# sttts/kcp

Measured on AMD Instinct MI355X. Metric: object-pair diffs/sec (whole node) + achieved HBM GB/s, 10M objs/100k clusters, higher is better.
Workload: dtype u8; 1 GPU; config3: 10000000 pairs / 100000 logical clusters node-wide, 5% mutated (40% ConfigMap/Secret, 40% Deployment, 20% CRD); pairs_per_rank=10000000, passes_in_flight=2, parallelism=shard-by-logical-cluster x1 (LPT)

## Files before the change

include/gpudiff.h:

```cpp
#ifndef GPUDIFF_H
#define GPUDIFF_H

#include <stddef.h>
#include <stdint.h>

#include "gpudiff_format.h"

#ifdef __cplusplus
extern "C" {
#endif

#define GPUDIFF_ABI_VERSION 6

enum {
    GPUDIFF_OK = 0,
    GPUDIFF_E_INVAL = -1,
    GPUDIFF_E_NOMEM = -2,
    GPUDIFF_E_DEVICE = -3,
    GPUDIFF_E_NODEVICE = -4,
    GPUDIFF_E_CAPACITY = -5,
    GPUDIFF_E_STATE = -6,
    GPUDIFF_E_DECODE = -7,
    GPUDIFF_E_NOTFOUND = -8,
};
// ... 166 lines not shown
int gpudiff_dbatch_create(gpudiff_ctx* ctx, uint64_t pool_bytes, uint64_t max_pairs,
                          gpudiff_dbatch** out);
int gpudiff_dbatch_create_view(gpudiff_ctx* ctx, const gpudiff_dbatch* base, gpudiff_dbatch** out);
int gpudiff_dbatch_append(gpudiff_ctx* ctx, gpudiff_dbatch* db, const gpudiff_hbatch* hb);
int gpudiff_dbatch_reset(gpudiff_ctx* ctx, gpudiff_dbatch* db);
int gpudiff_dbatch_stats_get(const gpudiff_dbatch* db, gpudiff_batch_stats* st);
int gpudiff_dbatch_device_view(const gpudiff_dbatch* db, gpudiff_device_view* v);
#define GPUDIFF_EXPORT_COUNTS 0u
#define GPUDIFF_EXPORT_SPEC_IDS 1u
#define GPUDIFF_EXPORT_STATUS_IDS 2u
#define GPUDIFF_EXPORT_DIRTY_IDS 3u
#define GPUDIFF_EXPORT_FLAGS 4u
int gpudiff_dbatch_export(gpudiff_ctx* ctx, const gpudiff_dbatch* db, uint32_t what, void* dst_device,
                          uint64_t max_elems, uint64_t known_count);
int gpudiff_dbatch_bind_gather(gpudiff_ctx* ctx, gpudiff_dbatch* db, void* send_dev, uint32_t cap_spec,
                               uint32_t cap_status);
int gpudiff_dbatch_result_slot(gpudiff_ctx* ctx, gpudiff_dbatch* db, uint32_t slot);
int gpudiff_dbatch_read_pool(gpudiff_ctx* ctx, const gpudiff_dbatch* db, uint64_t off, void* dst,
                             uint64_t bytes);
void gpudiff_dbatch_free(gpudiff_ctx* ctx, gpudiff_dbatch* db);

int gpudiff_cluster_bytes(const gpudiff_pair_row* rows, size_t n, uint32_t n_clusters, uint64_t* out);
int gpudiff_shard_lpt(const uint64_t* weights, uint32_t n_clusters, uint32_t world, int32_t* owner);

int gpudiff_diff(gpudiff_ctx* ctx, gpudiff_dbatch* db, gpudiff_ticket* ticket);
int gpudiff_wait(gpudiff_ctx* ctx, gpudiff_ticket ticket, gpudiff_result* res);
void gpudiff_result_release(gpudiff_ctx* ctx, gpudiff_result* res);
int gpudiff_last_timings(gpudiff_ctx* ctx, gpudiff_timings* t);
int gpudiff_timing_reset(gpudiff_ctx* ctx);
int gpudiff_sync(gpudiff_ctx* ctx);
typedef struct gpudiff_pass_stats {
    uint64_t passes;
    uint64_t small_passes;
    uint64_t small_redone;
    uint64_t redo_arena, redo_deep, redo_paths;
    uint64_t readback_rounds;
} gpudiff_pass_stats;
int gpudiff_pass_stats_get(gpudiff_ctx* ctx, gpudiff_pass_stats* out);

int gpudiff_submit(gpudiff_ctx* ctx, const gpudiff_json_pair* pairs, size_t n,
                   gpudiff_ticket* ticket);

typedef struct gpudiff_store gpudiff_store;

typedef struct gpudiff_event {
    uint32_t slot;
// ... 220 lines not shown
```

include/gpudiff_format.h:

```cpp
#ifndef GPUDIFF_FORMAT_H
#define GPUDIFF_FORMAT_H

#include <stdint.h>

#ifdef __HIPCC__
#define GPUDIFF_HD __host__ __device__
#else
#define GPUDIFF_HD
#endif

#define GPUDIFF_TAG_NULL 0u
#define GPUDIFF_TAG_FALSE 1u
#define GPUDIFF_TAG_TRUE 2u
#define GPUDIFF_TAG_INT 3u
#define GPUDIFF_TAG_FLOAT 4u
#define GPUDIFF_TAG_STR 5u
#define GPUDIFF_TAG_EOBJ 6u
#define GPUDIFF_TAG_EARR 7u

#define GPUDIFF_INLINE_MAX 8u
#define GPUDIFF_PATH_HASH_BITS 32u

#define GPUDIFF_OBJ_HAS_STATUS 0x1u
#define GPUDIFF_OBJ_DECODE_ERR 0x2u
#define GPUDIFF_OBJ_FRESH 0x4u
#define GPUDIFF_TAB_INDEX 0x8000000000000000ull
#define GPUDIFF_TAB_NONE 0xFFFFFFFFu
GPUDIFF_HD static inline uint64_t gpudiff_tab_bytes(uint32_t n, uint64_t key_bytes) {
    return (24ull * n + key_bytes + 127u) & ~(uint64_t)127u;
}

#define GPUDIFF_OBJ_SEED_SHIFT 8u

#ifdef __cplusplus
extern "C" {
#endif

typedef struct gpudiff_pair_row {
    uint64_t off_a;
    uint64_t off_b;
    uint32_t spec_l_a, spec_l_b;
    uint32_t spec_ar_a, spec_ar_b;
    uint32_t stat_l_a, stat_l_b;
    uint32_t stat_ar_a, stat_ar_b;
    uint32_t flags_a, flags_b;
    uint32_t pair_id, cluster_id;
} gpudiff_pair_row;

GPUDIFF_HD static inline uint64_t gpudiff_seg_bytes(uint32_t l, uint32_t arena) {
    return (uint64_t)l * 16u + (uint64_t)arena;
}

#define GPUDIFF_BLOB_ALIGN 128u
GPUDIFF_HD static inline uint64_t gpudiff_blob_body(uint32_t sl, uint32_t sar, uint32_t tl, uint32_t tar) {
    return (gpudiff_seg_bytes(sl, sar) + gpudiff_seg_bytes(tl, tar) + (GPUDIFF_BLOB_ALIGN - 1u)) &
           ~(uint64_t)(GPUDIFF_BLOB_ALIGN - 1u);
}

GPUDIFF_HD static inline uint64_t gpudiff_pair_compare_bytes(const gpudiff_pair_row* r) {
    const uint64_t al = GPUDIFF_BLOB_ALIGN - 1u;
    uint64_t per = 0;
    if ((r->flags_a | r->flags_b) & GPUDIFF_OBJ_DECODE_ERR) return sizeof(gpudiff_pair_row) + 1u;
    {
        const int spec_sz = r->spec_l_a == r->spec_l_b && r->spec_ar_a == r->spec_ar_b;
        const int stat_sz = (r->flags_b & GPUDIFF_OBJ_HAS_STATUS) && r->stat_l_a == r->stat_l_b &&
                            r->stat_ar_a == r->stat_ar_b;
        const uint64_t seg_s = gpudiff_seg_bytes(r->spec_l_a, r->spec_ar_a);
        const uint64_t seg_t = gpudiff_seg_bytes(r->stat_l_a, r->stat_ar_a);
        if (spec_sz && stat_sz) per = (seg_s + seg_t + al) & ~al;
        else if (spec_sz) per = (r->stat_l_a | r->stat_l_b | r->stat_ar_a | r->stat_ar_b) ? seg_s : (seg_s + al) & ~al;
        else if (stat_sz) per = seg_t;
    }
    return sizeof(gpudiff_pair_row) + 1u + 2u * per;
}

#define GPUDIFF_PD_ERR 0x01u
#define GPUDIFF_PD_SPEC_EQ 0x02u
#define GPUDIFF_PD_STAT_EQ 0x04u
#define GPUDIFF_PD_HAS_ST_B 0x08u
#define GPUDIFF_PD_HAS_ST_A 0x10u
#define GPUDIFF_PD_SEED 0x20u
#define GPUDIFF_PD_NO_STAT 0x40u
#define GPUDIFF_PD_SIZE_BITS 19u
#define GPUDIFF_PD_SIZE_MAX 0x7FFFFu
#define GPUDIFF_PD_ESCAPE 0xFFFFFFFFu

typedef struct gpudiff_pair_desc {
    uint32_t w[4];
} gpudiff_pair_desc;

typedef struct gpudiff_pair_geom {
    uint64_t off_a, off_b;
    uint32_t n1, n2, adj_a, adj_b;
    uint32_t bits;
} gpudiff_pair_geom;

GPUDIFF_HD static inline gpudiff_pair_geom gpudiff_pair_geom_of(uint64_t off_a, uint64_t off_b, uint32_t seg_a,
                                                                uint32_t seg_b, uint32_t seg_t, uint32_t bits) {
    gpudiff_pair_geom g;
    const int ok = !(bits & GPUDIFF_PD_ERR);
    const int spec_sz = (bits & GPUDIFF_PD_SPEC_EQ) != 0u;
    const int stat_sz = (bits & GPUDIFF_PD_HAS_ST_B) && (bits & GPUDIFF_PD_STAT_EQ);
    const uint32_t r128 = (seg_a + seg_t + 127u) & ~127u;
    g.off_a = off_a;
    g.off_b = off_b;
    g.n1 = (ok && spec_sz) ? ((!stat_sz && (bits & GPUDIFF_PD_NO_STAT)) ? ((seg_a + 127u) & ~127u) : seg_a) >> 4 : 0u;
    g.n2 = (ok && stat_sz) ? (spec_sz ? r128 - seg_a : seg_t) >> 4 : 0u;
    g.adj_a = seg_a - 16u * g.n1;
    g.adj_b = seg_b - 16u * g.n1;
    g.bits = bits;
    return g;
}

GPUDIFF_HD static inline uint32_t gpudiff_pair_row_bits(const gpudiff_pair_row* r) {
    return (((r->flags_a | r->flags_b) & GPUDIFF_OBJ_DECODE_ERR) ? GPUDIFF_PD_ERR : 0u) |
           ((r->spec_l_a == r->spec_l_b && r->spec_ar_a == r->spec_ar_b) ? GPUDIFF_PD_SPEC_EQ : 0u) |
           ((r->stat_l_a == r->stat_l_b && r->stat_ar_a == r->stat_ar_b) ? GPUDIFF_PD_STAT_EQ : 0u) |
           ((r->flags_b & GPUDIFF_OBJ_HAS_STATUS) ? GPUDIFF_PD_HAS_ST_B : 0u) |
           ((r->flags_a & GPUDIFF_OBJ_HAS_STATUS) ? GPUDIFF_PD_HAS_ST_A : 0u) |
           (((r->flags_a >> GPUDIFF_OBJ_SEED_SHIFT) & 0xFFu) ? GPUDIFF_PD_SEED : 0u) |
           ((r->stat_l_a | r->stat_l_b | r->stat_ar_a | r->stat_ar_b) == 0u ? GPUDIFF_PD_NO_STAT : 0u);
}

GPUDIFF_HD static inline gpudiff_pair_geom gpudiff_pair_row_geom(const gpudiff_pair_row* r) {
    return gpudiff_pair_geom_of(r->off_a, r->off_b, (uint32_t)gpudiff_seg_bytes(r->spec_l_a, r->spec_ar_a),
                                (uint32_t)gpudiff_seg_bytes(r->spec_l_b, r->spec_ar_b),
                                (uint32_t)gpudiff_seg_bytes(r->stat_l_a, r->stat_ar_a), gpudiff_pair_row_bits(r));
}

GPUDIFF_HD static inline gpudiff_pair_desc gpudiff_pair_desc_pack(const gpudiff_pair_row* r) {
    gpudiff_pair_desc d;
    const uint64_t sa = gpudiff_seg_bytes(r->spec_l_a, r->spec_ar_a), sb = gpudiff_seg_bytes(r->spec_l_b, r->spec_ar_b);
    const uint64_t st = gpudiff_seg_bytes(r->stat_l_a, r->stat_ar_a);
    const uint32_t bits = gpudiff_pair_row_bits(r);
    const uint64_t size_max = (uint64_t)GPUDIFF_PD_SIZE_MAX << 4;
    const int fits = ((r->off_a | r->off_b) & (GPUDIFF_BLOB_ALIGN - 1u)) == 0u && (r->off_a >> 7) <= 0xFFFFFFFFull &&
                     (r->off_b >> 7) <= 0xFFFFFFFFull && ((sa | sb | st) & 15u) == 0u && sa <= size_max &&
                     sb <= size_max && st <= size_max &&
                     ((uint32_t)(r->stat_l_a + r->stat_l_b) == 0u) == ((bits & GPUDIFF_PD_NO_STAT) != 0u);
    if (!fits) {
        d.w[0] = d.w[1] = d.w[2] = d.w[3] = GPUDIFF_PD_ESCAPE;
        return d;
    }
    {
        const uint64_t zw = (sa >> 4) | ((sb >> 4) << GPUDIFF_PD_SIZE_BITS) | ((st >> 4) << (2u * GPUDIFF_PD_SIZE_BITS)) |
                            ((uint64_t)bits << (3u * GPUDIFF_PD_SIZE_BITS));
        d.w[0] = (uint32_t)(r->off_a >> 7);
        d.w[1] = (uint32_t)(r->off_b >> 7);
        d.w[2] = (uint32_t)zw;
        d.w[3] = (uint32_t)(zw >> 32);
    }
    return d;
}

GPUDIFF_HD static inline int gpudiff_pair_desc_is_escape(uint32_t w3) { return w3 == GPUDIFF_PD_ESCAPE; }

GPUDIFF_HD static inline gpudiff_pair_geom gpudiff_pair_desc_unpack(uint32_t w0, uint32_t w1, uint32_t w2, uint32_t w3) {
    const uint64_t zw = ((uint64_t)w3 << 32) | w2;
    return gpudiff_pair_geom_of((uint64_t)w0 << 7, (uint64_t)w1 << 7, (w2 & GPUDIFF_PD_SIZE_MAX) << 4,
                                ((uint32_t)(zw >> GPUDIFF_PD_SIZE_BITS) & GPUDIFF_PD_SIZE_MAX) << 4,
                                ((w3 >> (2u * GPUDIFF_PD_SIZE_BITS - 32u)) & GPUDIFF_PD_SIZE_MAX) << 4,
                                w3 >> (3u * GPUDIFF_PD_SIZE_BITS - 32u));
}

GPUDIFF_HD static inline uint32_t gpudiff_meta(uint32_t tag, uint32_t len) { return (len << 3) | tag; }
GPUDIFF_HD static inline uint32_t gpudiff_meta_tag(uint32_t m) { return m & 7u; }
GPUDIFF_HD static inline uint32_t gpudiff_meta_len(uint32_t m) { return m >> 3; }
GPUDIFF_HD static inline int gpudiff_meta_is_long(uint32_t m) {
    return gpudiff_meta_tag(m) == GPUDIFF_TAG_STR && gpudiff_meta_len(m) > GPUDIFF_INLINE_MAX;
}
GPUDIFF_HD static inline uint32_t gpudiff_meta_arena(uint32_t m) {
    return gpudiff_meta_is_long(m) ? ((gpudiff_meta_len(m) - GPUDIFF_INLINE_MAX + 3u) & ~3u) : 0u;
}
GPUDIFF_HD static inline uint32_t gpudiff_arena_bytes(uint32_t sum) { return (sum + 15u) & ~15u; }

#ifdef __cplusplus
}
#endif
#endif
```

kcp_amd/csrc/api.cpp:

```cpp
#include <hip/hip_runtime.h>
#include <stdlib.h>
#include <string.h>

#include <algorithm>
#include <array>
#include <atomic>
#include <memory>
#include <mutex>
#include <new>
#include <string>
#include <thread>
#include <unordered_map>
#include <vector>

#include "../../include/gpudiff.h"
#include "encoder.h"
#include "dstore.h"
#include "engine.h"
#include "kernels.h"
#include "small_pass.h"
#include "xxh64.h"

using namespace gd;

// ... 543 lines not shown
    d->res_slot = slot;
    return GPUDIFF_OK;
}

int gpudiff_dbatch_read_pool(gpudiff_ctx* c, const gpudiff_dbatch* d, uint64_t off, void* dst, uint64_t bytes) {
    if (!c || !d || (!dst && bytes)) return GPUDIFF_E_INVAL;
    if (d->base) d = d->base;
    int rc = set_device(c);
    if (rc) return rc;
    if (off > d->pool_used || bytes > d->pool_used - off) return GPUDIFF_E_INVAL;
    HIPCHK(hipStreamSynchronize(c->stream));
    if (bytes) HIPCHK(hipMemcpy(dst, d->pool + off, bytes, hipMemcpyDeviceToHost));
    return GPUDIFF_OK;
}

int gpudiff_cluster_bytes(const gpudiff_pair_row* rows, size_t n, uint32_t n_clusters, uint64_t* out) {
    if ((n && !rows) || (n_clusters && !out)) return GPUDIFF_E_INVAL;
    for (size_t i = 0; i < n; i++)
        if (rows[i].cluster_id >= n_clusters) return GPUDIFF_E_INVAL;
    for (size_t i = 0; i < n; i++) out[rows[i].cluster_id] += gpudiff_pair_compare_bytes(&rows[i]);
    return GPUDIFF_OK;
}

int gpudiff_shard_lpt(const uint64_t* weights, uint32_t n_clusters, uint32_t world, int32_t* owner) {
    if (world == 0 || world > 0x7FFFFFFFu || (n_clusters && (!weights || !owner))) return GPUDIFF_E_INVAL;
    try {
        std::vector<uint32_t> order(n_clusters);
        for (uint32_t c = 0; c < n_clusters; c++) order[c] = c;
        std::sort(order.begin(), order.end(), [&](uint32_t x, uint32_t y) {
            return weights[x] != weights[y] ? weights[x] > weights[y] : x < y;
        });
        std::vector<std::pair<uint64_t, uint32_t>> heap;
        heap.reserve(world);
        for (uint32_t r = 0; r < world; r++) heap.emplace_back(0, r);
        auto gt = [](const std::pair<uint64_t, uint32_t>& a, const std::pair<uint64_t, uint32_t>& b) { return a > b; };
        std::make_heap(heap.begin(), heap.end(), gt);
        for (uint32_t c : order) {
            std::pop_heap(heap.begin(), heap.end(), gt);
            auto& top = heap.back();
            owner[c] = (int32_t)top.second;
            top.first += weights[c];
            std::push_heap(heap.begin(), heap.end(), gt);
        }
    } catch (const std::bad_alloc&) {
        return GPUDIFF_E_NOMEM;
    }
// ... 498 lines not shown
```

kcp_amd/csrc/encoder.cpp:

```cpp
#include "encoder.h"

#include <string.h>

#include <algorithm>

#include "xxh64.h"

namespace gd {

static const Node* find_member(const Node& obj, const char* key, uint32_t klen) {
    if (obj.t != J_OBJ) return nullptr;
    for (uint32_t i = 0; i < obj.n; i++) {
        const Member& m = obj.u.mem[i];
        if (m.klen == klen && memcmp(m.k, key, klen) == 0) return &m.v;
    }
    return nullptr;
}

static inline void push_key(std::string& p, const char* k, uint32_t n) {
    char hdr[5];
    hdr[0] = 0x01;
    memcpy(hdr + 1, &n, 4);
    p.append(hdr, 5);
    p.append(k, n);
// ... 237 lines not shown
    seg(o.spec, sl, sar);
    seg(o.stat, tl, tar);
    pool_align(pool);
}

void PairEncoder::encode_flat(FlatObject* fa, FlatObject* fb, uint32_t pair_id, uint32_t cluster_id,
                              std::vector<uint8_t>& pool, gpudiff_pair_row& row) {
    memset(&row, 0, sizeof(row));
    row.pair_id = pair_id;
    row.cluster_id = cluster_id;
    uint32_t seed = 0;
    if (!fa || !fb || !assign_seed(*fa, *fb, &seed)) {
        decode_errors++;
        pool_align(pool);
        row.off_a = row.off_b = pool.size();
        row.flags_a = row.flags_b = GPUDIFF_OBJ_DECODE_ERR;
        return;
    }
    if (seed) reseeded++;
    write_blob(*fa, pool, &row.off_a, &row.spec_l_a, &row.spec_ar_a, &row.stat_l_a, &row.stat_ar_a);
    write_blob(*fb, pool, &row.off_b, &row.spec_l_b, &row.spec_ar_b, &row.stat_l_b, &row.stat_ar_b);
    row.flags_a = fa->flags | (seed << GPUDIFF_OBJ_SEED_SHIFT);
    row.flags_b = fb->flags | (seed << GPUDIFF_OBJ_SEED_SHIFT);
}

void PairEncoder::encode_nodes(const Node* a, const Node* b, uint32_t pair_id, uint32_t cluster_id,
                               std::vector<uint8_t>& pool, gpudiff_pair_row& row) {
    FlatObject* fa = nullptr;
    FlatObject* fb = nullptr;
    if (a && b) {
        flatten_object(*a, flat_a);
        flatten_object(*b, flat_b);
        fa = &flat_a;
        fb = &flat_b;
    }
    encode_flat(fa, fb, pair_id, cluster_id, pool, row);
}

void PairEncoder::encode_json(const uint8_t* a, size_t alen, const uint8_t* b, size_t blen, uint32_t pair_id,
                              uint32_t cluster_id, std::vector<uint8_t>& pool, gpudiff_pair_row& row) {
    arena_a.reset();
    arena_b.reset();
    Node na, nb;
    bool oka = a && parser.parse_object(a, alen, arena_a, &na) && !decodes_as_list(na);
    bool okb = oka && b && parser.parse_object(b, blen, arena_b, &nb) && !decodes_as_list(nb);
    encode_nodes(oka ? &na : nullptr, okb ? &nb : nullptr, pair_id, cluster_id, pool, row);
// ... 229 lines not shown
```

kcp_amd/csrc/kernels.hip:

```cpp
#include <hip/hip_runtime.h>
#include <stdint.h>

#include "../../include/gpudiff.h"
#include "join_dev.h"
#include "kernels.h"
#include "stream_paths.h"
#include "wave_dev.h"
#include "xxh64.h"

namespace gd {


constexpr uint32_t SCAN_TILE = 4096;

struct V4 {
    uint32_t x, y, z, w;
};
__device__ __forceinline__ uint32_t vadd(uint32_t a, uint32_t b) { return a + b; }
__device__ __forceinline__ V4 vadd(const V4& a, const V4& b) {
    return V4{a.x + b.x, a.y + b.y, a.z + b.z, sat_add(a.w, b.w)};
}
template <class V> __device__ __forceinline__ V vzero() { return V{}; }
__device__ __forceinline__ uint32_t vshfl(uint32_t v, uint32_t src) { return shfl32(v, src); }
__device__ __forceinline__ V4 vshfl(const V4& v, uint32_t src) {
// ... 65 lines not shown
    V run = vadd(vadd(wpre[0], wpre[1]), vadd(wpre[2], wpre[3]));
    if (base_in) run = vadd(run, *base_in);
    for (uint32_t w = 0; w < (t >> 6); w++) run = vadd(run, wsum[w]);
    const V excl_thread = vshfl(incl, lane_id() ? lane_id() - 1 : 0);
    if (lane_id()) run = vadd(run, excl_thread);
#pragma unroll
    for (int k = 0; k < 16; k++) {
        const uint32_t i = base + t * 16 + k;
        if (i < n) out[i] = run;
        run = vadd(run, v[k]);
    }
    if (blockIdx.x == last && t == 255) {
        *total = run;
        if (write_terminal) out[n] = run;
        if (mirror) mirror_store(mirror, run);
    }
}


struct StreamLog {
    uint32_t cnt[2][64];
    uint32_t ent[2][64][kSpLogCap];
    uint32_t first[64], n1[64];
};

__device__ uint32_t stream_region(const RegionView& A, const RegionView& B, uint64_t seg, const uint32_t* ent,
                                  uint32_t c, uint32_t g0, uint8_t region_bit, uint64_t* __restrict__ out_h,
                                  uint8_t* __restrict__ out_k, uint32_t out_base, uint32_t lane, bool* weq_all) {
    const uint32_t nc = 4u * c;
    const uint32_t e = lane < nc ? ent[lane >> 2] - sp_entry(g0, 0u) : 0u;
    const bool cand = lane < nc && ((sp_entry_dwords(e) >> (lane & 3u)) & 1u);
    const uint64_t b = sp_entry_byte(e, lane & 3u);
    const SpWhere w = sp_classify(b, A.L);
    if (ballot(cand && (b >= seg || w.cls == SP_KEY))) return kSpRefuse;
    uint32_t leaf = w.idx;
    const bool ar = cand && w.cls == SP_ARENA;
    if (ballot(ar)) {
        bool found = false;
        uint32_t run = 0;
        for (uint32_t i0 = 0; i0 < A.L; i0 += 64u) {
            const uint32_t n = min(64u, A.L - i0);
            const uint32_t as = lane < n ? meta_arena(A.metas[i0 + lane]) : 0u;
            const uint32_t inc = wave_incl_scan(as);
            const uint32_t tot = shfl32(inc, 63);
            const uint32_t rel = w.idx - run;
            uint32_t o = 0;
#pragma unroll
            for (uint32_t s = 32; s >= 1; s >>= 1)
                if (shfl32(inc, o + s - 1u) <= rel) o += s;
            if (ar && !found && w.idx >= run && rel < tot) {
                leaf = i0 + o;
                found = true;
            }
// ... 25 lines not shown
        xb = B.vals[leaf];
    }
    if (ballot(uq && meta_arena(ma) != meta_arena(mb))) return kSpRefuse;
    if (uq) {
        out_h[out_base + rank] = key;
        out_k[out_base + rank] = region_bit | GPUDIFF_PATH_CHANGED;
    }
    *weq_all = !ballot(uq && !wire_equal_number(ma, xa, mb, xb));
    return popc64(um);
}

__device__ uint32_t stream_pair(const gpudiff_pair_row& r, uint32_t f, const uint8_t* pool, uint64_t mask,
                                uint64_t* out_h, uint8_t* out_k, uint32_t base, uint32_t lane, uint32_t* noop,
                                const StreamLog* log, uint32_t k, bool log_ok, uint32_t* n_stream) {
    uint32_t n = 0;
    bool spec_weq = true, stat_weq = true;
    if (f & F_JSPEC) {
        RegionView A = region_view(pool, r.off_a, r.spec_l_a, r.spec_ar_a, false, r.spec_l_a);
        RegionView B = region_view(pool, r.off_b, r.spec_l_b, r.spec_ar_b, false, r.spec_l_b);
        const uint32_t c = log_ok ? uni(log->cnt[0][k]) : 0u;
        const uint32_t g0 = uni(log->first[k]);
        uint32_t got = kSpRefuse;
        if (c >= 1u && c <= kSpLogCap)
            got = stream_region(A, B, seg_bytes(r.spec_l_a, r.spec_ar_a), log->ent[0][k], c, g0, 0, out_h, out_k, base + n,
                                lane, &spec_weq);
        if (got == kSpRefuse) got = join_region<true>(A, B, 0, out_h, out_k, base + n, lane, &spec_weq);
        else (*n_stream)++;
        n += got;
    }
    if (f & F_JSTAT) {
        RegionView A = region_view(pool, r.off_a, r.spec_l_a, r.spec_ar_a, true, r.stat_l_a);
        RegionView B = region_view(pool, r.off_b, r.spec_l_b, r.spec_ar_b, true, r.stat_l_b);
        const uint32_t c = log_ok ? uni(log->cnt[1][k]) : 0u;
        const uint32_t g0 = uni(log->first[k]) + uni(log->n1[k]);
        uint32_t got = kSpRefuse;
        if (c >= 1u && c <= kSpLogCap)
            got = stream_region(A, B, seg_bytes(r.stat_l_a, r.stat_ar_a), log->ent[1][k], c, g0,
                                GPUDIFF_PATH_REGION_STATUS, out_h, out_k, base + n, lane, &stat_weq);
        if (got == kSpRefuse)
            got = join_region<true>(A, B, GPUDIFF_PATH_REGION_STATUS, out_h, out_k, base + n, lane, &stat_weq);
        else (*n_stream)++;
        n += got;
    }
    const bool stat_ok = stat_weq && (!(f & F_SENT) || !(r.flags_a & GPUDIFF_OBJ_HAS_STATUS));
    *noop = (((f & F_SPEC) && spec_weq) ? NOOP_SPEC : 0u) | (((f & F_STATUS) && stat_ok) ? NOOP_STATUS : 0u);
    if (f & F_SENT) {
        if (lane == 0) {
            out_h[base + n] = status_sentinel_hash((r.flags_a >> GPUDIFF_OBJ_SEED_SHIFT) & 0xFFu, mask);
            out_k[base + n] = GPUDIFF_PATH_REGION_STATUS | GPUDIFF_PATH_STATUS_ABSENT;
        }
        n += 1;
    }
    return n;
}

__device__ __forceinline__ bool place_deferred(uint32_t d, uint64_t so, uint32_t cap, uint64_t scratch_cap,
                                               uint32_t* __restrict__ slot_owner) {
    if (so > scratch_cap || cap > scratch_cap - so) return false;
    const uint32_t b0 = (uint32_t)((so + kJoinSlice - 1u) / kJoinSlice);
    const uint32_t b1 = (uint32_t)((so + cap + kJoinSlice - 1u) / kJoinSlice);
// ... 361 lines not shown
    const uint32_t nwaves = (gridDim.x * blockDim.x) >> 6;
    const uint32_t sub_shift = sub_arg & 0xFFu, tail_q = (sub_arg >> 8) & 0xFFu;
    const uint32_t tail_ish = min(sub_shift + 1u, 3u);
    const uint32_t wbase = arena_off + wave * arena_stride;
    uint32_t used = 0;
    bool deferred = false;
    const uint64_t sent0 = status_sentinel_hash(0, mask);
    __shared__ HelpSlot help_slots[HELP ? 4 : 1];
    [[maybe_unused]] HelpSlot* const my = &help_slots[HELP ? (threadIdx.x >> 6) : 0];
    if constexpr (HELP) {
        if (lane == 0) {
            my->gen = my->cursor = my->total = my->helpers = my->p0 = my->cnt = 0u;
            my->mis_s = my->mis_t = 0ull;
        }
        __syncthreads();
    }
    [[maybe_unused]] StreamLog* slog = nullptr;
    [[maybe_unused]] uint32_t n_stream = 0;
    if constexpr (!HELP) {
        __shared__ StreamLog stream_logs[4];
        slog = &stream_logs[uni(threadIdx.x >> 6)];
    }
    auto stream_pass = [&](uint32_t base, uint32_t total, uint32_t incl, uint32_t first, uint32_t n1, uint32_t adj_a,
                           uint32_t adj_b, uint64_t off_a, uint64_t off_b, uint64_t& mis_s, uint64_t& mis_t) {
        u32x4 va[U], vb[U];
        uint32_t own[U];
        bool st[U], act[U];
#pragma unroll
        for (int u = 0; u < U; u++) {
            const uint32_t g = base + (uint32_t)u * 64u + lane;
            act[u] = g < total;
            uint32_t o = 0;
#pragma unroll
            for (uint32_t s = 32; s >= 1; s >>= 1)
                if (shfl32(incl, o + s - 1u) <= g) o += s;
            const uint32_t k = g - shfl32(first, o);
            st[u] = k >= shfl32(n1, o);
            const uint32_t xa = shfl32(adj_a, o), xb = shfl32(adj_b, o);
            const uint64_t oa = shfl64(off_a, o), ob = shfl64(off_b, o);
            own[u] = HELP ? o : o | (st[u] ? 64u : 0u);
            const uint64_t rel = 16ull * k;
            if (act[u]) {
                va[u] = __builtin_nontemporal_load((const u32x4*)(pool + oa + rel + (st[u] ? xa : 0u)));
                vb[u] = __builtin_nontemporal_load((const u32x4*)(pool + ob + rel + (st[u] ? xb : 0u)));
            }
        }
        if constexpr (HELP) {
#pragma unroll
            for (int u = 0; u < U; u++) {
                uint64_t m = ballot(act[u] && neq16(va[u], vb[u]));
                while (m) {
                    const uint32_t j = (uint32_t)__builtin_ctzll(m);
                    m &= m - 1;
                    const uint64_t bit = 1ull << (uint32_t)__builtin_amdgcn_readlane((int)own[u], (int)j);
                    if (__builtin_amdgcn_readlane((int)(st[u] ? 1 : 0), (int)j)) mis_t |= bit;
                    else mis_s |= bit;
                }
            }
        } else {
            uint32_t info[U];
#pragma unroll
            for (int u = 0; u < U; u++) {
                const uint32_t dw = (va[u].x != vb[u].x ? 1u : 0u) | (va[u].y != vb[u].y ? 2u : 0u) |
                                    (va[u].z != vb[u].z ? 4u : 0u) | (va[u].w != vb[u].w ? 8u : 0u);
                info[u] = own[u] | (act[u] ? dw << 7 : 0u);
            }
#pragma unroll
// ... 68 lines not shown
            if (!HELP && it < n_main && lane == 0) tk = atomicAdd(ctr, 1u);
            continue;
        }
        const uint32_t cnt = min(per, n - p0);
        const bool valid = lane < cnt;
        u32x4 v0 = {0, 0, 0, 0}, v1 = v0, v2 = v0, v3 = v0;
        [[maybe_unused]] u32x4 dv = v0;
        if constexpr (DESC) {
            if (valid) dv = *(const u32x4*)(desc + p0 + lane);
        } else if (valid) {
            const u32x4* rp = (const u32x4*)(rows + p0 + lane);
            v0 = rp[0];
            v1 = rp[1];
            v2 = rp[2];
            v3 = rp[3];
        }
        if constexpr (PROF) {
            tp_r = wall_clock64();
            tp_rows += tp_r - tp_i;
        }
        uint64_t off_a, off_b;
        bool err, spec_sz, has_st_b, stat_sz;
        uint32_t n1, n2, adj_a, adj_b;
        [[maybe_unused]] uint32_t dbits = 0;
        constexpr uint32_t kPdRow = 0x80u;
        if constexpr (DESC) {
            gpudiff_pair_geom g = gpudiff_pair_desc_unpack(dv.x, dv.y, dv.z, dv.w);
            if (valid && gpudiff_pair_desc_is_escape(dv.w)) {
                const gpudiff_pair_row r = rows[p0 + lane];
                g = gpudiff_pair_row_geom(&r);
                g.bits |= kPdRow;
            }
            dbits = g.bits;
            off_a = g.off_a, off_b = g.off_b;
            err = valid && (dbits & GPUDIFF_PD_ERR) != 0u;
            spec_sz = (dbits & GPUDIFF_PD_SPEC_EQ) != 0u;
            has_st_b = (dbits & GPUDIFF_PD_HAS_ST_B) != 0u;
            stat_sz = has_st_b && (dbits & GPUDIFF_PD_STAT_EQ) != 0u;
            n1 = valid ? g.n1 : 0u, n2 = valid ? g.n2 : 0u;
            adj_a = g.adj_a, adj_b = g.adj_b;
        } else {
            off_a = ((uint64_t)v0.y << 32) | v0.x, off_b = ((uint64_t)v0.w << 32) | v0.z;
            err = valid && ((v3.x | v3.y) & GPUDIFF_OBJ_DECODE_ERR) != 0u;
            const bool ok = valid && !err;
            spec_sz = v1.x == v1.y && v1.z == v1.w;
            has_st_b = (v3.y & GPUDIFF_OBJ_HAS_STATUS) != 0u;
            stat_sz = has_st_b && v2.x == v2.y && v2.z == v2.w;
            const uint32_t seg_a = (uint32_t)seg_bytes(v1.x, v1.z), seg_b = (uint32_t)seg_bytes(v1.y, v1.w);
            const uint32_t seg_t = (uint32_t)seg_bytes(v2.x, v2.z);
            const uint32_t r128 = ((seg_a + seg_t + 127u) & ~127u);
            const bool no_stat = (v2.x | v2.y | v2.z | v2.w) == 0u;
            n1 = (ok && spec_sz) ? ((!stat_sz && no_stat) ? ((seg_a + 127u) & ~127u) : seg_a) >> 4 : 0u;
            n2 = (ok && stat_sz) ? (spec_sz ? r128 - seg_a : seg_t) >> 4 : 0u;
            adj_a = seg_a - 16u * n1, adj_b = seg_b - 16u * n1;
        }
        const uint32_t tot = n1 + n2;
        const uint32_t incl = wave_incl_scan(tot);
        const uint32_t total = uni(shfl32(incl, 63));
        const uint32_t first = incl - tot;
        uint64_t mis_s = 0, mis_t = 0;
        [[maybe_unused]] uint64_t tp_s0 = 0;
        if constexpr (PROF) {
            tp_s0 = wall_clock64();
// ... 10 lines not shown
                __hip_atomic_store(&my->mis_t, 0ull, __ATOMIC_RELAXED, __HIP_MEMORY_SCOPE_WORKGROUP);
                lds_st(&my->cursor, 64u * U);
                lds_st(&my->gen, lds_ld(&my->gen) + 1u);
            }
            for (uint32_t base = 0; base < total;) {
                uint32_t nb = 0;
                if (lane == 0) nb = lds_add(&my->cursor, 64u * U);
                stream_pass(base, total, incl, first, n1, adj_a, adj_b, off_a, off_b, mis_s, mis_t);
                base = uni(__builtin_amdgcn_readlane(nb, 0));
            }
            if (lane == 0) {
                lds_or64(&my->mis_s, mis_s);
                lds_or64(&my->mis_t, mis_t);
            }
            while (uni(lds_ld(&my->helpers)) != 0u) __builtin_amdgcn_s_sleep(1);
            const uint64_t ms = lds_ld64(&my->mis_s), mt = lds_ld64(&my->mis_t);
            mis_s = ((uint64_t)uni((uint32_t)(ms >> 32)) << 32) | uni((uint32_t)ms);
            mis_t = ((uint64_t)uni((uint32_t)(mt >> 32)) << 32) | uni((uint32_t)mt);
        } else {
            slog->cnt[0][lane] = 0u;
            slog->cnt[1][lane] = 0u;
            slog->first[lane] = first;
            slog->n1[lane] = n1;
            uint32_t pass = 0;
            for (uint32_t base = 0; base < total; base += 64u * U, pass++) {
                stream_pass(base, total, incl, first, n1, adj_a, adj_b, off_a, off_b, mis_s, mis_t);
                if (pass == 0 && it < n_main && lane == 0) tk = atomicAdd(ctr, 1u);
            }
            if (pass == 0 && it < n_main && lane == 0) tk = atomicAdd(ctr, 1u);
        }
        [[maybe_unused]] uint64_t tp_s1 = 0;
        if constexpr (PROF) {
            tp_s1 = wall_clock64();
            tp_stream += tp_s1 - tp_s0;
        }
        if constexpr (DESC) {
            v3.x = ((dbits & GPUDIFF_PD_HAS_ST_A) ? GPUDIFF_OBJ_HAS_STATUS : 0u) |
                   ((dbits & GPUDIFF_PD_SEED) ? 1u << GPUDIFF_OBJ_SEED_SHIFT : 0u);
            const bool sd = !spec_sz || ((mis_s >> lane) & 1ull), td = !stat_sz || ((mis_t >> lane) & 1ull);
            const bool plain_sent = !sd && !has_st_b && (dbits & GPUDIFF_PD_NO_STAT) && !(dbits & (GPUDIFF_PD_SEED | kPdRow));
            if (valid && !err && (sd || td) && !plain_sent) {
                const uint32_t* rp = (const uint32_t*)(rows + p0 + lane);
                const uint2 ls = *(const uint2*)(rp + 4), lt = *(const uint2*)(rp + 8);
                v1.x = ls.x, v1.y = ls.y;
                v2.x = lt.x, v2.y = lt.y;
                v3.x = rp[12];
            }
        }
        uint32_t myflag = 0, mycap = 0, mysrc = 0, mycnt = 0, mynoop = 0;
// ... 516 lines not shown
```

kcp_amd/csrc/stream_paths.h:

```cpp
#pragma once
#include <stdint.h>

#include "../../include/gpudiff_format.h"

#if defined(__HIPCC__)
#define GD_SP_HD __host__ __device__
#else
#define GD_SP_HD
#endif

namespace gd {

constexpr uint32_t kSpLogCap = 4;
constexpr uint32_t kSpMaxLeaves = 64;
constexpr uint32_t kSpRefuse = 0xFFFFFFFFu;

GD_SP_HD inline uint32_t sp_entry(uint32_t chunk, uint32_t dwords) { return (chunk << 4) | (dwords & 15u); }
GD_SP_HD inline uint32_t sp_entry_dwords(uint32_t e) { return e & 15u; }
GD_SP_HD inline uint64_t sp_entry_byte(uint32_t e, uint32_t d) { return 16ull * (e >> 4) + 4u * d; }

GD_SP_HD inline uint32_t sp_meta_arena(uint32_t m) {
    return ((m & 7u) == GPUDIFF_TAG_STR && (m >> 3) > GPUDIFF_INLINE_MAX) ? (((m >> 3) - GPUDIFF_INLINE_MAX + 3u) & ~3u)
                                                                          : 0u;
}

enum SpClass : uint32_t { SP_VAL = 0, SP_KEY = 1, SP_META = 2, SP_ARENA = 3 };
struct SpWhere {
    uint32_t cls;
    uint32_t idx;
};
GD_SP_HD inline SpWhere sp_classify(uint64_t b, uint32_t L) {
    const uint64_t l = L;
    if (b < 8u * l) return SpWhere{SP_VAL, (uint32_t)(b >> 3)};
    if (b < 12u * l) return SpWhere{SP_KEY, (uint32_t)((b - 8u * l) >> 2)};
    if (b < 16u * l) return SpWhere{SP_META, (uint32_t)((b - 12u * l) >> 2)};
    return SpWhere{SP_ARENA, (uint32_t)(b - 16u * l)};
}

GD_SP_HD inline uint32_t sp_arena_owner(const uint32_t* metas, uint32_t L, uint32_t ao) {
    uint32_t off = 0;
    for (uint32_t i = 0; i < L; i++) {
        const uint32_t n = sp_meta_arena(metas[i]);
// ... 35 lines not shown
```

kcp_amd/gpudiff.py:

```python
from __future__ import annotations

import ctypes as C
import json
import os
from dataclasses import dataclass
from typing import Any, Iterable, List, Optional, Sequence, Tuple, Union

import numpy as np

from . import buildinfo

_HERE = os.path.dirname(os.path.abspath(__file__))
LIB_PATH = os.path.join(_HERE, "libgpudiff.so")

ABI_VERSION = 6
OK = 0
E_INVAL, E_NOMEM, E_DEVICE, E_NODEVICE, E_CAPACITY, E_STATE, E_DECODE, E_NOTFOUND = range(-1, -9, -1)

SPEC_DIRTY, STATUS_DIRTY, DECODE_ERROR, SPEC_NOOP, STATUS_NOOP = 0x1, 0x2, 0x4, 0x8, 0x10
PATH_CHANGED, PATH_ADDED, PATH_REMOVED, PATH_STATUS_ABSENT = 0, 1, 2, 3
PATH_REGION_STATUS = 0x80
TAG_NULL, TAG_FALSE, TAG_TRUE, TAG_INT, TAG_FLOAT, TAG_STR, TAG_EOBJ, TAG_EARR = range(8)
VALUE_ABSENT = 0xFF
OPT_TIMING = 0x1
OPT_DEVICE_ENCODE = 0x2000000
OPT_PATH_STRINGS = 0x8000000
OPT_PATH_VALUES = 0x80000000
OPT_K2_ROWS = 0x40
OPT_ARENA_SHIFT = 21
OPT_SMALL_PASS = 0x20000000
SMALL_PASS_MAX_PAIRS = 4096
SMALL_PASS_MAX_PATHS = 32768
DEVICE_CURRENT, DEVICE_NONE = -1, -2

PATH_HASH_BITS = 32
OBJ_HAS_STATUS, OBJ_DECODE_ERR, OBJ_FRESH, OBJ_SEED_SHIFT = 0x1, 0x2, 0x4, 8
STORE_DEVICE_ENCODE = 0x1
EXPORT_COUNTS, EXPORT_SPEC_IDS, EXPORT_STATUS_IDS, EXPORT_DIRTY_IDS, EXPORT_FLAGS = range(5)


class GpuDiffError(RuntimeError):
    def __init__(self, code: int, where: str):
        self.code = code
        super().__init__("%s: %s (%d)" % (where, _lib.gpudiff_strerror(code).decode(), code))


class Opts(C.Structure):
    _fields_ = [("device", C.c_int32), ("encode_threads", C.c_uint32), ("stream", C.c_void_p),
                ("flags", C.c_uint32), ("path_hash_bits", C.c_uint32)]


class JsonPair(C.Structure):
    _fields_ = [("old_json", C.c_void_p), ("old_len", C.c_size_t), ("new_json", C.c_void_p),
                ("new_len", C.c_size_t), ("pair_id", C.c_uint32), ("cluster_id", C.c_uint32)]


JSON_PAIR_DTYPE = np.dtype([("old_json", "<u8"), ("old_len", "<u8"), ("new_json", "<u8"), ("new_len", "<u8"),
                            ("pair_id", "<u4"), ("cluster_id", "<u4")])
assert JSON_PAIR_DTYPE.itemsize == C.sizeof(JsonPair)
# ... 241 lines not shown
SIGNATURES = [
    ("gpudiff_strerror", C.c_char_p, [C.c_int]),
    ("gpudiff_abi_version", C.c_int, []),
    ("gpudiff_build_id", C.c_char_p, []),
    ("gpudiff_device_count", C.c_int, [C.POINTER(C.c_int)]),
    ("gpudiff_open", C.c_int, [C.POINTER(Opts), C.POINTER(_P)]),
    ("gpudiff_close", None, [_P]),
    ("gpudiff_encode_pairs", C.c_int, [_P, C.POINTER(JsonPair), C.c_size_t, C.POINTER(_P)]),
    ("gpudiff_hbatch_info_get", C.c_int, [_P, C.POINTER(HBatchInfo)]),
    ("gpudiff_hbatch_free", None, [_P, _P]),
    ("gpudiff_dbatch_create", C.c_int, [_P, C.c_uint64, C.c_uint64, C.POINTER(_P)]),
    ("gpudiff_dbatch_append", C.c_int, [_P, _P, _P]),
    ("gpudiff_dbatch_reset", C.c_int, [_P, _P]),
    ("gpudiff_dbatch_stats_get", C.c_int, [_P, C.POINTER(BatchStats)]),
    ("gpudiff_dbatch_device_view", C.c_int, [_P, C.POINTER(DeviceView)]),
    ("gpudiff_dbatch_read_pool", C.c_int, [_P, _P, C.c_uint64, C.c_void_p, C.c_uint64]),
    ("gpudiff_dbatch_export", C.c_int, [_P, _P, C.c_uint32, C.c_void_p, C.c_uint64, C.c_uint64]),
    ("gpudiff_dbatch_free", None, [_P, _P]),
    ("gpudiff_dbatch_bind_gather", C.c_int, [_P, _P, C.c_void_p, C.c_uint32, C.c_uint32]),
    ("gpudiff_dbatch_result_slot", C.c_int, [_P, _P, C.c_uint32]),
    ("gpudiff_dbatch_create_view", C.c_int, [_P, _P, C.POINTER(_P)]),
    ("gpudiff_cluster_bytes", C.c_int, [C.c_void_p, C.c_size_t, C.c_uint32, C.c_void_p]),
    ("gpudiff_shard_lpt", C.c_int, [C.c_void_p, C.c_uint32, C.c_uint32, C.c_void_p]),
    ("gpudiff_diff", C.c_int, [_P, _P, C.POINTER(C.c_uint64)]),
    ("gpudiff_wait", C.c_int, [_P, C.c_uint64, C.POINTER(Result)]),
    ("gpudiff_result_release", None, [_P, C.POINTER(Result)]),
    ("gpudiff_result_path_strings", C.c_int, [_P, C.POINTER(Result), C.POINTER(PathStringsC)]),
    ("gpudiff_path_strings_stats_get", C.c_int, [_P, C.POINTER(PathStats)]),
    ("gpudiff_result_path_values", C.c_int, [_P, C.POINTER(Result), C.POINTER(PathValuesC)]),
    ("gpudiff_path_values_stats_get", C.c_int, [_P, C.POINTER(PathStats)]),
    ("gpudiff_render_syncs_get", C.c_int, [_P, C.POINTER(C.c_uint64)]),
    ("gpudiff_render_value_from_blob", C.c_int, [C.c_char_p, C.POINTER(ObjInfo), C.c_uint32, C.c_uint64,
                                                 C.POINTER(C.c_uint8), C.c_void_p, C.c_size_t, C.POINTER(C.c_size_t)]),
    ("gpudiff_last_timings", C.c_int, [_P, C.POINTER(Timings)]),
    ("gpudiff_pass_stats_get", C.c_int, [_P, C.POINTER(PassStats)]),
    ("gpudiff_sync", C.c_int, [_P]),
    ("gpudiff_timing_reset", C.c_int, [_P]),
    ("gpudiff_hbatch_create", C.c_int, [_P, C.c_uint64, C.c_size_t, C.c_uint64, C.POINTER(_P), C.POINTER(_P),
                                        C.POINTER(_P)]),
    ("gpudiff_hbatch_resize", C.c_int, [_P, _P, C.c_uint64, C.c_size_t, C.c_uint64, C.POINTER(_P),
                                        C.POINTER(_P)]),
    ("gpudiff_submit", C.c_int, [_P, C.POINTER(JsonPair), C.c_size_t, C.POINTER(C.c_uint64)]),
    ("gpudiff_store_create", C.c_int, [_P, C.c_uint32, C.c_uint64, C.c_uint32, C.POINTER(_P)]),
    ("gpudiff_store_create_ex", C.c_int, [_P, C.c_uint32, C.c_uint64, C.c_uint32, C.c_uint32, C.POINTER(_P)]),
    ("gpudiff_store_submit", C.c_int, [_P, _P, C.POINTER(Event), C.c_size_t, C.POINTER(C.c_uint64)]),
    ("gpudiff_store_forget", C.c_int, [_P, _P, C.c_uint32]),
# ... 98 lines not shown

def lib() -> C.CDLL:
    return _lib


def _chk(rc: int, where: str):
    if rc != OK:
        raise GpuDiffError(rc, where)


def device_count() -> int:
    n = C.c_int(0)
    _chk(_lib.gpudiff_device_count(C.byref(n)), "gpudiff_device_count")
    return n.value


def cluster_bytes(rows: np.ndarray, n_clusters: int) -> np.ndarray:
    rows = np.ascontiguousarray(rows, dtype=ROW_DTYPE)
    out = np.zeros(n_clusters, dtype=np.uint64)
    _chk(_lib.gpudiff_cluster_bytes(rows.ctypes.data, rows.size, n_clusters, out.ctypes.data), "gpudiff_cluster_bytes")
    return out


def shard_lpt(weights, world: int) -> np.ndarray:
    w = np.ascontiguousarray(weights, dtype=np.uint64)
    owner = np.zeros(w.size, dtype=np.int32)
    _chk(_lib.gpudiff_shard_lpt(w.ctypes.data, w.size, world, owner.ctypes.data), "gpudiff_shard_lpt")
    return owner


def to_json_bytes(obj: Union[bytes, bytearray, str, dict]) -> bytes:
    if isinstance(obj, (bytes, bytearray)):
        return bytes(obj)
    if isinstance(obj, str):
        return obj.encode()
    return json.dumps(obj, separators=(",", ":")).encode()


@dataclass
class DiffResult:
    pair_flags: np.ndarray
    spec_dirty_ids: np.ndarray
    status_dirty_ids: np.ndarray
    dirty_ids: np.ndarray
    path_offsets: np.ndarray
    path_hashes: np.ndarray
# ... 898 lines not shown
```

Measured before the change: 1.238 billion pairs/s.

## Skip streaming the key-hash region of spec when both objects share identical keys

The encoder now marks pairs whose spec key hashes match, and the packed descriptor carries a hole covering the key-hash portion of the spec segment. The streaming compare kernel skips those 128-byte lines when loading A and B and remaps stream-log entries around the hole. This cuts HBM bytes read per equal-layout pair, at the cost of an extra per-pair key comparison in the host encoder and more index arithmetic in the kernel. It also adds an API that counts streamed bytes, and it folds adj_b into off_b.

```diff
diff --git a/include/gpudiff.h b/include/gpudiff.h
--- a/include/gpudiff.h
+++ b/include/gpudiff.h
@@ -212,6 +212,7 @@
 
 int gpudiff_cluster_bytes(const gpudiff_pair_row* rows, size_t n, uint32_t n_clusters, uint64_t* out);
 int gpudiff_shard_lpt(const uint64_t* weights, uint32_t n_clusters, uint32_t world, int32_t* owner);
+int gpudiff_rows_stream_bytes(const gpudiff_pair_row* rows, size_t n, uint64_t* out);
 
 int gpudiff_diff(gpudiff_ctx* ctx, gpudiff_dbatch* db, gpudiff_ticket* ticket);
 int gpudiff_wait(gpudiff_ctx* ctx, gpudiff_ticket ticket, gpudiff_result* res);
diff --git a/include/gpudiff_format.h b/include/gpudiff_format.h
--- a/include/gpudiff_format.h
+++ b/include/gpudiff_format.h
@@ -24,6 +24,7 @@
 #define GPUDIFF_OBJ_HAS_STATUS 0x1u
 #define GPUDIFF_OBJ_DECODE_ERR 0x2u
 #define GPUDIFF_OBJ_FRESH 0x4u
+#define GPUDIFF_OBJ_SPEC_KEYS_EQ 0x8u
 #define GPUDIFF_TAB_INDEX 0x8000000000000000ull
 #define GPUDIFF_TAB_NONE 0xFFFFFFFFu
 GPUDIFF_HD static inline uint64_t gpudiff_tab_bytes(uint32_t n, uint64_t key_bytes) {
@@ -55,6 +56,19 @@
 GPUDIFF_HD static inline uint64_t gpudiff_blob_body(uint32_t sl, uint32_t sar, uint32_t tl, uint32_t tar) {
     return (gpudiff_seg_bytes(sl, sar) + gpudiff_seg_bytes(tl, tar) + (GPUDIFF_BLOB_ALIGN - 1u)) &
            ~(uint64_t)(GPUDIFF_BLOB_ALIGN - 1u);
+}
+
+#ifndef GPUDIFF_KEYS_HOLE_UNIT
+#define GPUDIFF_KEYS_HOLE_UNIT 128u
+#endif
+GPUDIFF_HD static inline void gpudiff_keys_hole(uint32_t l, uint32_t* hs, uint32_t* hl) {
+    const uint64_t u = GPUDIFF_KEYS_HOLE_UNIT;
+    const uint64_t lo = (8ull * l + (u - 1u)) / u * u, hi = 12ull * l / u * u;
+    *hs = hi > lo ? (uint32_t)(lo >> 4) : 0u;
+    *hl = hi > lo ? (uint32_t)((hi - lo) >> 4) : 0u;
+}
+GPUDIFF_HD static inline uint32_t gpudiff_hole_chunk(uint32_t k, uint32_t hs, uint32_t hl) {
+    return k + (k >= hs ? hl : 0u);
 }
 
 GPUDIFF_HD static inline uint64_t gpudiff_pair_compare_bytes(const gpudiff_pair_row* r) {
@@ -93,10 +107,12 @@
     uint64_t off_a, off_b;
     uint32_t n1, n2, adj_a, adj_b;
     uint32_t bits;
+    uint32_t hs, hl;
 } gpudiff_pair_geom;
 
 GPUDIFF_HD static inline gpudiff_pair_geom gpudiff_pair_geom_of(uint64_t off_a, uint64_t off_b, uint32_t seg_a,
-                                                                uint32_t seg_b, uint32_t seg_t, uint32_t bits) {
+                                                                uint32_t seg_b, uint32_t seg_t, uint32_t bits,
+                                                                uint32_t skip_l) {
     gpudiff_pair_geom g;
     const int ok = !(bits & GPUDIFF_PD_ERR);
     const int spec_sz = (bits & GPUDIFF_PD_SPEC_EQ) != 0u;
@@ -106,6 +122,11 @@
     g.off_b = off_b;
     g.n1 = (ok && spec_sz) ? ((!stat_sz && (bits & GPUDIFF_PD_NO_STAT)) ? ((seg_a + 127u) & ~127u) : seg_a) >> 4 : 0u;
     g.n2 = (ok && stat_sz) ? (spec_sz ? r128 - seg_a : seg_t) >> 4 : 0u;
+    g.hs = g.hl = 0u;
+    if (skip_l && (uint64_t)skip_l * 12u <= 16ull * g.n1) {
+        gpudiff_keys_hole(skip_l, &g.hs, &g.hl);
+        g.n1 -= g.hl;
+    }
     g.adj_a = seg_a - 16u * g.n1;
     g.adj_b = seg_b - 16u * g.n1;
     g.bits = bits;
@@ -125,7 +146,7 @@
 GPUDIFF_HD static inline gpudiff_pair_geom gpudiff_pair_row_geom(const gpudiff_pair_row* r) {
     return gpudiff_pair_geom_of(r->off_a, r->off_b, (uint32_t)gpudiff_seg_bytes(r->spec_l_a, r->spec_ar_a),
                                 (uint32_t)gpudiff_seg_bytes(r->spec_l_b, r->spec_ar_b),
-                                (uint32_t)gpudiff_seg_bytes(r->stat_l_a, r->stat_ar_a), gpudiff_pair_row_bits(r));
+                                (uint32_t)gpudiff_seg_bytes(r->stat_l_a, r->stat_ar_a), gpudiff_pair_row_bits(r), 0u);
 }
 
 GPUDIFF_HD static inline gpudiff_pair_desc gpudiff_pair_desc_pack(const gpudiff_pair_row* r) {
@@ -143,7 +164,13 @@
         return d;
     }
     {
-        const uint64_t zw = (sa >> 4) | ((sb >> 4) << GPUDIFF_PD_SIZE_BITS) | ((st >> 4) << (2u * GPUDIFF_PD_SIZE_BITS)) |
+        uint64_t f1 = sb >> 4;
+        if (bits & GPUDIFF_PD_SPEC_EQ) {
+            uint32_t hs = 0, hl = 0;
+            if ((r->flags_b & GPUDIFF_OBJ_SPEC_KEYS_EQ) && !(bits & GPUDIFF_PD_ERR)) gpudiff_keys_hole(r->spec_l_a, &hs, &hl);
+            f1 = hl ? r->spec_l_a : 0u;
+        }
+        const uint64_t zw = (sa >> 4) | (f1 << GPUDIFF_PD_SIZE_BITS) | ((st >> 4) << (2u * GPUDIFF_PD_SIZE_BITS)) |
                             ((uint64_t)bits << (3u * GPUDIFF_PD_SIZE_BITS));
         d.w[0] = (uint32_t)(r->off_a >> 7);
         d.w[1] = (uint32_t)(r->off_b >> 7);
@@ -157,10 +184,20 @@
 
 GPUDIFF_HD static inline gpudiff_pair_geom gpudiff_pair_desc_unpack(uint32_t w0, uint32_t w1, uint32_t w2, uint32_t w3) {
     const uint64_t zw = ((uint64_t)w3 << 32) | w2;
-    return gpudiff_pair_geom_of((uint64_t)w0 << 7, (uint64_t)w1 << 7, (w2 & GPUDIFF_PD_SIZE_MAX) << 4,
-                                ((uint32_t)(zw >> GPUDIFF_PD_SIZE_BITS) & GPUDIFF_PD_SIZE_MAX) << 4,
-                                ((w3 >> (2u * GPUDIFF_PD_SIZE_BITS - 32u)) & GPUDIFF_PD_SIZE_MAX) << 4,
-                                w3 >> (3u * GPUDIFF_PD_SIZE_BITS - 32u));
+    const uint32_t bits = w3 >> (3u * GPUDIFF_PD_SIZE_BITS - 32u);
+    const uint32_t seg_a = (w2 & GPUDIFF_PD_SIZE_MAX) << 4;
+    const uint32_t f1 = (uint32_t)(zw >> GPUDIFF_PD_SIZE_BITS) & GPUDIFF_PD_SIZE_MAX;
+    const int eq = (bits & GPUDIFF_PD_SPEC_EQ) != 0u;
+    return gpudiff_pair_geom_of((uint64_t)w0 << 7, (uint64_t)w1 << 7, seg_a, eq ? seg_a : f1 << 4,
+                                ((w3 >> (2u * GPUDIFF_PD_SIZE_BITS - 32u)) & GPUDIFF_PD_SIZE_MAX) << 4, bits,
+                                eq ? f1 : 0u);
+}
+
+GPUDIFF_HD static inline uint64_t gpudiff_pair_stream_bytes(const gpudiff_pair_row* r) {
+    const gpudiff_pair_desc d = gpudiff_pair_desc_pack(r);
+    const gpudiff_pair_geom g = gpudiff_pair_desc_is_escape(d.w[3]) ? gpudiff_pair_row_geom(r)
+                                                                   : gpudiff_pair_desc_unpack(d.w[0], d.w[1], d.w[2], d.w[3]);
+    return sizeof(gpudiff_pair_desc) + 32ull * ((uint64_t)g.n1 + g.n2);
 }
 
 GPUDIFF_HD static inline uint32_t gpudiff_meta(uint32_t tag, uint32_t len) { return (len << 3) | tag; }
diff --git a/kcp_amd/csrc/api.cpp b/kcp_amd/csrc/api.cpp
--- a/kcp_amd/csrc/api.cpp
+++ b/kcp_amd/csrc/api.cpp
@@ -589,6 +589,14 @@
     return GPUDIFF_OK;
 }
 
+int gpudiff_rows_stream_bytes(const gpudiff_pair_row* rows, size_t n, uint64_t* out) {
+    if ((n && !rows) || !out) return GPUDIFF_E_INVAL;
+    uint64_t sum = 0;
+    for (size_t i = 0; i < n; i++) sum += gpudiff_pair_stream_bytes(&rows[i]);
+    *out = sum;
+    return GPUDIFF_OK;
+}
+
 int gpudiff_shard_lpt(const uint64_t* weights, uint32_t n_clusters, uint32_t world, int32_t* owner) {
     if (world == 0 || world > 0x7FFFFFFFu || (n_clusters && (!weights || !owner))) return GPUDIFF_E_INVAL;
     try {
diff --git a/kcp_amd/csrc/encoder.cpp b/kcp_amd/csrc/encoder.cpp
--- a/kcp_amd/csrc/encoder.cpp
+++ b/kcp_amd/csrc/encoder.cpp
@@ -283,6 +283,9 @@
     write_blob(*fb, pool, &row.off_b, &row.spec_l_b, &row.spec_ar_b, &row.stat_l_b, &row.stat_ar_b);
     row.flags_a = fa->flags | (seed << GPUDIFF_OBJ_SEED_SHIFT);
     row.flags_b = fb->flags | (seed << GPUDIFF_OBJ_SEED_SHIFT);
+    bool keys_eq = fa->spec.size() == fb->spec.size();
+    for (size_t i = 0; keys_eq && i < fa->spec.size(); i++) keys_eq = (uint32_t)fa->spec[i].h == (uint32_t)fb->spec[i].h;
+    if (keys_eq) row.flags_b |= GPUDIFF_OBJ_SPEC_KEYS_EQ;
 }
 
 void PairEncoder::encode_nodes(const Node* a, const Node* b, uint32_t pair_id, uint32_t cluster_id,
diff --git a/kcp_amd/csrc/kernels.hip b/kcp_amd/csrc/kernels.hip
--- a/kcp_amd/csrc/kernels.hip
+++ b/kcp_amd/csrc/kernels.hip
@@ -111,13 +111,15 @@
     uint32_t cnt[2][64];
     uint32_t ent[2][64][kSpLogCap];
     uint32_t first[64], n1[64];
+    uint32_t hole[64];
 };
 
 __device__ uint32_t stream_region(const RegionView& A, const RegionView& B, uint64_t seg, const uint32_t* ent,
-                                  uint32_t c, uint32_t g0, uint8_t region_bit, uint64_t* __restrict__ out_h,
-                                  uint8_t* __restrict__ out_k, uint32_t out_base, uint32_t lane, bool* weq_all) {
+                                  uint32_t c, uint32_t g0, uint32_t hole, uint8_t region_bit,
+                                  uint64_t* __restrict__ out_h, uint8_t* __restrict__ out_k, uint32_t out_base,
+                                  uint32_t lane, bool* weq_all) {
     const uint32_t nc = 4u * c;
-    const uint32_t e = lane < nc ? ent[lane >> 2] - sp_entry(g0, 0u) : 0u;
+    const uint32_t e = lane < nc ? sp_entry_unhole(ent[lane >> 2] - sp_entry(g0, 0u), hole) : 0u;
     const bool cand = lane < nc && ((sp_entry_dwords(e) >> (lane & 3u)) & 1u);
     const uint64_t b = sp_entry_byte(e, lane & 3u);
     const SpWhere w = sp_classify(b, A.L);
@@ -189,8 +191,8 @@
         const uint32_t g0 = uni(log->first[k]);
         uint32_t got = kSpRefuse;
         if (c >= 1u && c <= kSpLogCap)
-            got = stream_region(A, B, seg_bytes(r.spec_l_a, r.spec_ar_a), log->ent[0][k], c, g0, 0, out_h, out_k, base + n,
-                                lane, &spec_weq);
+            got = stream_region(A, B, seg_bytes(r.spec_l_a, r.spec_ar_a), log->ent[0][k], c, g0, uni(log->hole[k]), 0,
+                                out_h, out_k, base + n, lane, &spec_weq);
         if (got == kSpRefuse) got = join_region<true>(A, B, 0, out_h, out_k, base + n, lane, &spec_weq);
         else (*n_stream)++;
         n += got;
@@ -202,7 +204,7 @@
         const uint32_t g0 = uni(log->first[k]) + uni(log->n1[k]);
         uint32_t got = kSpRefuse;
         if (c >= 1u && c <= kSpLogCap)
-            got = stream_region(A, B, seg_bytes(r.stat_l_a, r.stat_ar_a), log->ent[1][k], c, g0,
+            got = stream_region(A, B, seg_bytes(r.stat_l_a, r.stat_ar_a), log->ent[1][k], c, g0, 0u,
                                 GPUDIFF_PATH_REGION_STATUS, out_h, out_k, base + n, lane, &stat_weq);
         if (got == kSpRefuse)
             got = join_region<true>(A, B, GPUDIFF_PATH_REGION_STATUS, out_h, out_k, base + n, lane, &stat_weq);
@@ -610,7 +612,8 @@
         slog = &stream_logs[uni(threadIdx.x >> 6)];
     }
     auto stream_pass = [&](uint32_t base, uint32_t total, uint32_t incl, uint32_t first, uint32_t n1, uint32_t adj_a,
-                           uint32_t adj_b, uint64_t off_a, uint64_t off_b, uint64_t& mis_s, uint64_t& mis_t) {
+                           uint32_t adj_b, uint64_t off_a, uint64_t off_b, uint64_t& mis_s, uint64_t& mis_t,
+                           [[maybe_unused]] uint32_t hole = 0u) {
         u32x4 va[U], vb[U];
         uint32_t own[U];
         bool st[U], act[U];
@@ -624,13 +627,18 @@
                 if (shfl32(incl, o + s - 1u) <= g) o += s;
             const uint32_t k = g - shfl32(first, o);
             st[u] = k >= shfl32(n1, o);
-            const uint32_t xa = shfl32(adj_a, o), xb = shfl32(adj_b, o);
+            const uint32_t xa = shfl32(adj_a, o), xb = DESC ? xa : shfl32(adj_b, o);
             const uint64_t oa = shfl64(off_a, o), ob = shfl64(off_b, o);
             own[u] = HELP ? o : o | (st[u] ? 64u : 0u);
             const uint64_t rel = 16ull * k;
+            uint32_t ha = 0;
+            if constexpr (DESC) {
+                const uint32_t hw = shfl32(hole, o);
+                ha = k >= sp_hole_start(hw) ? sp_hole_bytes(hw) : 0u;
+            }
             if (act[u]) {
-                va[u] = __builtin_nontemporal_load((const u32x4*)(pool + oa + rel + (st[u] ? xa : 0u)));
-                vb[u] = __builtin_nontemporal_load((const u32x4*)(pool + ob + rel + (st[u] ? xb : 0u)));
+                va[u] = __builtin_nontemporal_load((const u32x4*)(pool + oa + rel + (st[u] ? xa : ha)));
+                vb[u] = __builtin_nontemporal_load((const u32x4*)(pool + ob + rel + (st[u] ? xb : ha)));
             }
         }
         if constexpr (HELP) {
@@ -745,6 +753,7 @@
         uint64_t off_a, off_b;
         bool err, spec_sz, has_st_b, stat_sz;
         uint32_t n1, n2, adj_a, adj_b;
+        [[maybe_unused]] uint32_t hole = 0;
         [[maybe_unused]] uint32_t dbits = 0;
         constexpr uint32_t kPdRow = 0x80u;
         if constexpr (DESC) {
@@ -761,7 +770,9 @@
             has_st_b = (dbits & GPUDIFF_PD_HAS_ST_B) != 0u;
             stat_sz = has_st_b && (dbits & GPUDIFF_PD_STAT_EQ) != 0u;
             n1 = valid ? g.n1 : 0u, n2 = valid ? g.n2 : 0u;
-            adj_a = g.adj_a, adj_b = g.adj_b;
+            off_b += (uint64_t)g.adj_b - (uint64_t)g.adj_a;
+            adj_a = adj_b = g.adj_a;
+            hole = sp_hole_word(g.hs, g.hl);
         } else {
             off_a = ((uint64_t)v0.y << 32) | v0.x, off_b = ((uint64_t)v0.w << 32) | v0.z;
             err = valid && ((v3.x | v3.y) & GPUDIFF_OBJ_DECODE_ERR) != 0u;
@@ -818,9 +829,10 @@
             slog->cnt[1][lane] = 0u;
             slog->first[lane] = first;
             slog->n1[lane] = n1;
+            slog->hole[lane] = hole;
             uint32_t pass = 0;
             for (uint32_t base = 0; base < total; base += 64u * U, pass++) {
-                stream_pass(base, total, incl, first, n1, adj_a, adj_b, off_a, off_b, mis_s, mis_t);
+                stream_pass(base, total, incl, first, n1, adj_a, adj_b, off_a, off_b, mis_s, mis_t, hole);
                 if (pass == 0 && it < n_main && lane == 0) tk = atomicAdd(ctr, 1u);
             }
             if (pass == 0 && it < n_main && lane == 0) tk = atomicAdd(ctr, 1u);
diff --git a/kcp_amd/csrc/stream_paths.h b/kcp_amd/csrc/stream_paths.h
--- a/kcp_amd/csrc/stream_paths.h
+++ b/kcp_amd/csrc/stream_paths.h
@@ -18,6 +18,15 @@
 GD_SP_HD inline uint32_t sp_entry(uint32_t chunk, uint32_t dwords) { return (chunk << 4) | (dwords & 15u); }
 GD_SP_HD inline uint32_t sp_entry_dwords(uint32_t e) { return e & 15u; }
 GD_SP_HD inline uint64_t sp_entry_byte(uint32_t e, uint32_t d) { return 16ull * (e >> 4) + 4u * d; }
+
+static_assert(GPUDIFF_KEYS_HOLE_UNIT % 128u == 0u, "sp_hole_word keeps the hole in 128-B lines");
+GD_SP_HD inline uint32_t sp_hole_word(uint32_t hs, uint32_t hl) { return (hs >> 3) | ((hl >> 3) << 16); }
+GD_SP_HD inline uint32_t sp_hole_start(uint32_t w) { return (w & 0xFFFFu) << 3; }
+GD_SP_HD inline uint32_t sp_hole_chunks(uint32_t w) { return (w >> 16) << 3; }
+GD_SP_HD inline uint32_t sp_hole_bytes(uint32_t w) { return (w >> 16) << 7; }
+GD_SP_HD inline uint32_t sp_entry_unhole(uint32_t e, uint32_t w) {
+    return e + ((e >> 4) >= sp_hole_start(w) ? sp_entry(sp_hole_chunks(w), 0u) : 0u);
+}
 
 GD_SP_HD inline uint32_t sp_meta_arena(uint32_t m) {
     return ((m & 7u) == GPUDIFF_TAG_STR && (m >> 3) > GPUDIFF_INLINE_MAX) ? (((m >> 3) - GPUDIFF_INLINE_MAX + 3u) & ~3u)
diff --git a/kcp_amd/gpudiff.py b/kcp_amd/gpudiff.py
--- a/kcp_amd/gpudiff.py
+++ b/kcp_amd/gpudiff.py
@@ -35,6 +35,7 @@
 
 PATH_HASH_BITS = 32
 OBJ_HAS_STATUS, OBJ_DECODE_ERR, OBJ_FRESH, OBJ_SEED_SHIFT = 0x1, 0x2, 0x4, 8
+OBJ_SPEC_KEYS_EQ = 0x8
 STORE_DEVICE_ENCODE = 0x1
 EXPORT_COUNTS, EXPORT_SPEC_IDS, EXPORT_STATUS_IDS, EXPORT_DIRTY_IDS, EXPORT_FLAGS = range(5)
 
@@ -322,6 +323,7 @@
     ("gpudiff_dbatch_create_view", C.c_int, [_P, _P, C.POINTER(_P)]),
     ("gpudiff_cluster_bytes", C.c_int, [C.c_void_p, C.c_size_t, C.c_uint32, C.c_void_p]),
     ("gpudiff_shard_lpt", C.c_int, [C.c_void_p, C.c_uint32, C.c_uint32, C.c_void_p]),
+    ("gpudiff_rows_stream_bytes", C.c_int, [C.c_void_p, C.c_size_t, C.POINTER(C.c_uint64)]),
     ("gpudiff_diff", C.c_int, [_P, _P, C.POINTER(C.c_uint64)]),
     ("gpudiff_wait", C.c_int, [_P, C.c_uint64, C.POINTER(Result)]),
     ("gpudiff_result_release", None, [_P, C.POINTER(Result)]),
@@ -466,6 +468,13 @@
     return out
 
 
+def stream_bytes(rows: np.ndarray) -> int:
+    rows = np.ascontiguousarray(rows, dtype=ROW_DTYPE)
+    out = C.c_uint64()
+    _chk(_lib.gpudiff_rows_stream_bytes(rows.ctypes.data, rows.size, C.byref(out)), "gpudiff_rows_stream_bytes")
+    return int(out.value)
+
+
 def shard_lpt(weights, world: int) -> np.ndarray:
     w = np.ascontiguousarray(weights, dtype=np.uint64)
     owner = np.zeros(w.size, dtype=np.int32)
```

After: 1.296 billion pairs/s (median of 6 runs). 4.7% higher.
